# rubengooj/pl-slam

Measured on AMD Instinct MI355X. Metric: stereo pairs/sec (1500 ORB + 200 LBD BF-match), higher is better.
Workload: dtype fp4; 1 GPU; C2: synthetic 752x480 stereo stream, 1500 ORB + 200 LBD per image, ORB+LBD L<->R and prev<->curr, mutual + ratio (StVO::match), then StereoFrame's gates over the L<->R tables (config_kitti.yaml:25-...; mutual=True, distinct_batches_in_rotation=3, stereo_gates=True, kernel=k_scan_sym_mfma_i, mfma_form=0

## Files before the change

plslam_amd/build.py:

```python
from __future__ import annotations

import hashlib
import os
import shutil
import subprocess
from concurrent.futures import ThreadPoolExecutor

_HERE = os.path.dirname(os.path.abspath(__file__))
_ROOT = os.path.dirname(_HERE)
CSRC = os.path.join(_HERE, "csrc")
OUT = os.path.join(_HERE, "lib", "libplslam_hip.so")
LEGACY_OUT = os.path.join(_HERE, "lib", "libplslam_hip_legacy.so")
OBJ_DIR = os.path.join(_ROOT, "build", "obj")
SOURCES = ["hamming.hip", "hamming_mfma_g.hip", "hamming_mfma_h.hip", "hamming_mfma_i.hip", "lba.hip", "lba_assemble_rows.hip", "lba_plan.hip", "lba_schur.hip",
           "map2kf.hip", "lbd.hip", "median_desc.hip", "match_grid.hip", "match_grid_listers.hip", "match_grid_dense.hip", "match_grid_api.hip", "stereo_gates.hip", "pose_gn.hip", "lbd_float.hip", "bow.hip",
           "loop_closure.hip", "gba.hip", "pgo.hip", "local_map.hip", "map_insert.hip", "lc_fuse.hip",
           "context.hip", "match_plan.hip", "host_calls.hip", "match_pipeline.hip", "gather.hip"]
LEGACY_SOURCES = ["hamming_mfma.hip", "hamming_mfma_d.hip"]
LEGACY_AWARE = ("context.hip", "hamming_mfma_h.hip")
HEADERS = [os.path.join(CSRC, h) for h in ("common.hpp", "match_tables.hpp", "match_planner.hpp", "match_plan.hpp", "gfx950_only.hpp", "mfma_h_common.hpp", "lba_rows_dev.hpp", "lba_lists.hpp", "lba_blocks_dev.hpp", "lba_plan.hpp", "match_grid.hpp", "match_grid_layout.hpp", "match_grid_dev.hpp",
                                            "stereo_gates_dev.hpp", "pose_gn_dev.hpp", "se3_dev.hpp", "ldlt_dense_dev.hpp", "lookback_dev.hpp", "lc_fuse_plan.hpp")] + [os.path.join(_ROOT, "include", "plslam_hip.h")]
FLAGS = ["--offload-arch=gfx950", "-O3", "-std=c++17", "-fPIC", "-ffp-contract=off",
         "-Wall", "-Wextra", "-Wno-unused-command-line-argument",
         "-include", os.path.join(CSRC, "gfx950_only.hpp")]
PER_SOURCE_FLAGS = {"hamming_mfma_h.hip": ["-Wno-inline-asm"], "hamming_mfma_i.hip": ["-Wno-inline-asm"]}


def legacy_scans() -> bool:
    return os.environ.get("PLSLAM_BUILD_LEGACY_SCANS", "0") not in ("", "0")
# ... 94 lines not shown
```

plslam_amd/csrc/common.hpp:

```cpp
#pragma once

#include <hip/hip_runtime.h>
#include <stdint.h>

#include <cstdio>
#include <mutex>
#include <vector>

#include "match_tables.hpp"
#include "plslam_hip.h"

namespace plslam {

void set_last_error(const char* fmt, ...);

#define PLSLAM_HIP_CHECK(expr)                                                              \
    do {                                                                                    \
        hipError_t e_ = (expr);                                                             \
        if (e_ != hipSuccess) {                                                             \
            ::plslam::set_last_error("%s:%d: %s -> %s", __FILE__, __LINE__, #expr,           \
                                     hipGetErrorString(e_));                                \
            return e_ == hipErrorOutOfMemory ? PLSLAM_ENOMEM : PLSLAM_EHIP;                 \
        }                                                                                   \
    } while (0)
// ... 95 lines not shown
    hipDeviceProp_t prop;
    int scan_variant = PLSLAM_SCAN_AUTO;
    int scan_block = 0;
    int group_cap = 0;
    int sym_rows = 0;
    int mfma_form = 0;
    int col_split = 0;
    int exact_second = 0;
    int graph = 1;
    int post_workgroups = 0;
    int split_target = 0, split_min_tiles = 0;
    int split_post = 0;
    int post_xcd = 2;
    int zero_copy_kb = 64;
    int post_fuse = 0;
    int fuse = 0;
    std::mutex mu;
    plslam::DevBuf in_a, in_b, out_a, out_b, misc_a, misc_b, misc_c;
    plslam::HostBuf pin_in, pin_out;
    plslam::HostBuf pin_misc;
    plslam::LineRing lbd_ring;
    struct plslam_match_plan* host_plan = nullptr;
    struct plslam_match_plan* lc_plan = nullptr;
    plslam::DevBuf lc_in, lc_out, lc_tab;
    hipEvent_t lc_ev[2] = {nullptr, nullptr};
    plslam::DevBuf lc_args;
    std::vector<char> lc_args_h;
    int pgo_solver = 0;
    plslam::DevBuf pgo_scratch;
};
// ... 51 lines not shown
int sym_rows_per_partial(int rows_per_lane);
int launch_scan_sym(int rows_per_lane, const SymDesc* d_sym, const BlockDesc* d_blocks, int nblocks,
                    int32_t* d_zero, int nzero, hipStream_t s);
int launch_scan_sym_mfma(const SymDesc* d_sym, const BlockDesc* d_blocks, int nblocks, int32_t* d_zero,
                         int nzero, bool multi_window, bool directed, hipStream_t s);
int launch_scan_sym_mfma_g(const SymDesc* d_sym, const BlockDesc* d_blocks, int nblocks, int32_t* d_zero,
                           int nzero, bool multi_window, bool directed, bool fused, hipStream_t s);
int merge_partials16_cols(int parts);
int launch_merge_partials16(const SymDesc* d_sym, const BlockDesc* d_blocks, int nblocks, int parts, hipStream_t s);
int launch_split_post(const SymDesc* d_sym, const BlockDesc* d_blocks, int nblocks, int parts, const ProblemDesc* d_probs, hipStream_t s);
int launch_split_rows_dump(const ProblemDesc* d_probs, const BlockDesc* d_fin_blocks, int nblocks, hipStream_t s);
int launch_scan_sym_mfma_h(const SymDesc* d_sym, const BlockDesc* d_blocks, int nblocks, int32_t* d_zero, int nzero,
                           bool directed, hipStream_t s);
int launch_scan_sym_mfma_i(const SymDesc* d_sym, const BlockDesc* d_blocks, int nblocks, int32_t* d_zero, int nzero,
                           bool directed, hipStream_t s);
int merge_fix16_cols(int parts);
int launch_merge_fix16(const SymDesc* d_sym, const BlockDesc* d_blocks, int nblocks, int parts, bool fix, hipStream_t s, int grid_cap = 0);
int mh_slot_of_column(int n2, int j);
int launch_scan_dir_mfma(const SymDesc* d_sym, const BlockDesc* d_blocks, int nblocks, int32_t* d_zero, int nzero, hipStream_t s);
int launch_scan_mfma_form(int form, const SymDesc* d_sym, const BlockDesc* d_blocks, int nblocks, int32_t* d_zero,
                          int nzero, bool multi_window, bool directed, hipStream_t s, bool fused = false);
int launch_merge_partials(const SymDesc* d_sym, const BlockDesc* d_blocks, int nblocks, hipStream_t s);

int scan_rows_per_block(int variant, int block_threads);

int launch_gather_rows(const void* src, const int32_t* idx, int32_t n, int32_t row_bytes, void* dst,
                       hipStream_t s);

int launch_point_rows(const plslam_cam& K, double th, const double* T, const double* Xw,
                      const double* uv, const int32_t* lm, const int32_t* kf, int32_t nobs,
// ... 25 lines not shown
```

plslam_amd/csrc/context.hip:

```cpp
#include <stdarg.h>
#include <string.h>

#include <new>

#include "common.hpp"
#include "match_grid.hpp"
#include "match_plan.hpp"

namespace plslam {

static thread_local char g_err[512] = "";

void set_last_error(const char* fmt, ...)
{
    va_list ap;
    va_start(ap, fmt);
    vsnprintf(g_err, sizeof(g_err), fmt, ap);
    va_end(ap);
}

int DevBuf::reserve(size_t bytes)
{
    if (bytes <= cap) return PLSLAM_OK;
    if (p) {
// ... 133 lines not shown
}

namespace {
int g_legacy_scans = PLSLAM_BUILD_LEGACY_SCANS;
struct OptionDesc { const char* name; int plslam_ctx::*member; int* global; int lo, hi; };
const OptionDesc kOptions[] = {
    {"scan_variant", &plslam_ctx::scan_variant, nullptr, PLSLAM_SCAN_AUTO, PLSLAM_SCAN_MFMA},
    {"scan_block", &plslam_ctx::scan_block, nullptr, 0, 1024},
    {"sym_rows", &plslam_ctx::sym_rows, nullptr, 0, 4},
    {"group_cap", &plslam_ctx::group_cap, nullptr, 0, 64},
    {"mfma_form", &plslam_ctx::mfma_form, nullptr, 0, 5},
    {"legacy_scans", nullptr, &g_legacy_scans, 0, -1},
    {"fuse", &plslam_ctx::fuse, nullptr, 0, 2},
    {"post_fuse", &plslam_ctx::post_fuse, nullptr, 0, 2},
    {"exact_second", &plslam_ctx::exact_second, nullptr, 0, 1},
    {"col_split", &plslam_ctx::col_split, nullptr, 0, 2},
    {"graph", &plslam_ctx::graph, nullptr, 0, 2},
    {"grid_dense", nullptr, &plslam::g_grid_dense, 0, 1},
    {"zero_copy_kb", &plslam_ctx::zero_copy_kb, nullptr, -(1 << 20), 1 << 20},
    {"post_xcd", &plslam_ctx::post_xcd, nullptr, 0, 2},
    {"split_post", &plslam_ctx::split_post, nullptr, 0, 1},
    {"split_target", &plslam_ctx::split_target, nullptr, 0, 64},
    {"split_min_tiles", &plslam_ctx::split_min_tiles, nullptr, 0, 64},
    {"post_workgroups", &plslam_ctx::post_workgroups, nullptr, 0, INT32_MAX},
    {"pgo_solver", &plslam_ctx::pgo_solver, nullptr, 0, 1},
};
const OptionDesc* find_option(const char* key, bool to_write)
{
    for (const OptionDesc& o : kOptions)
        if (!strcmp(key, o.name) && (!to_write || o.lo <= o.hi)) return &o;
// ... 46 lines not shown
```

plslam_amd/csrc/match_plan.hip:

```cpp
#include <string.h>

#include <new>

#include "match_plan.hpp"

using namespace plslam;

static PlanOptions plan_options_of(const plslam_ctx* ctx)
{
    PlanOptions o;
    o.cu_count = ctx->prop.multiProcessorCount;
    o.scan_variant = ctx->scan_variant; o.scan_block = ctx->scan_block; o.sym_rows = ctx->sym_rows; o.group_cap = ctx->group_cap;
    o.mfma_form = ctx->mfma_form; o.col_split = ctx->col_split; o.exact_second = ctx->exact_second;
    o.split_target = ctx->split_target; o.split_min_tiles = ctx->split_min_tiles; o.split_post = ctx->split_post;
    o.post_xcd = ctx->post_xcd; o.post_fuse = ctx->post_fuse; o.fuse = ctx->fuse;
    o.rows_wpq = scan_rows_per_block(PLSLAM_SCAN_WAVE_PER_QUERY, 256);
    o.rows_lpq = scan_rows_per_block(PLSLAM_SCAN_LANE_PER_QUERY, ctx->scan_block ? ctx->scan_block : 256);
    const int lanes[3] = {1, 4, 16};
    for (int k = 0; k < 3; ++k) { o.merge16_cols[k] = merge_partials16_cols(lanes[k]); o.fix16_cols[k] = merge_fix16_cols(lanes[k]); }
    for (int k = 0; k < 2; ++k) { o.sym_block_rows[k] = sym_rows_per_block(lanes[k]); o.sym_partial_rows[k] = sym_rows_per_partial(lanes[k]); }
    return o;
}

bool plslam::ctx_takes_device_row_count(const plslam_ctx* ctx) { return plan_options_of(ctx).takes_device_row_count(); }

int plslam::plan_build(plslam_ctx* ctx, const plslam_match_problem* probs, int32_t nprob,
                       plslam_match_plan* P, const int32_t* n1_dev0)
{
    PlanChoice& c = P->choice;
    PlanTables& t = P->tab;
// ... 30 lines not shown
    if (!base) {
        if ((r = P->tables.reserve(t.total))) return r;
        base = P->tables.as<char>();
    }
    auto at = [&](int k) { return base + t.piece[k].off; };
    P->d_scans = reinterpret_cast<ScanDesc*>(at(PlanTables::SCANS));
    P->d_syms = reinterpret_cast<SymDesc*>(at(PlanTables::SYMS));
    P->d_probs = reinterpret_cast<ProblemDesc*>(at(PlanTables::PROBS));
    P->d_scan_blocks = reinterpret_cast<BlockDesc*>(at(PlanTables::SCAN_BLOCKS));
    P->d_sym_blocks = reinterpret_cast<BlockDesc*>(at(PlanTables::SYM_BLOCKS));
    P->d_merge_blocks = reinterpret_cast<BlockDesc*>(at(PlanTables::MERGE_BLOCKS));
    P->d_fin_blocks = reinterpret_cast<BlockDesc*>(at(PlanTables::FIN_BLOCKS));
    P->d_count_dst = reinterpret_cast<int32_t**>(at(PlanTables::COUNT_DST));
    P->d_dirs = reinterpret_cast<SymDesc*>(at(PlanTables::DIRS));
    P->d_dir_blocks = reinterpret_cast<BlockDesc*>(at(PlanTables::DIR_BLOCKS));
    P->ngate_blocks = 0;
    P->ngates = 0;

    if (!P->probs_in_place) PLSLAM_HIP_CHECK(hipMemcpyAsync(base, stg, t.total, hipMemcpyHostToDevice, ctx->stream));
    return PLSLAM_OK;
}

int plslam::plan_run(plslam_match_plan* P, hipStream_t s, hipStream_t sp)
{
    const bool split = sp != s;
    if (split) {
        if (!P->scan_done) PLSLAM_HIP_CHECK(hipEventCreateWithFlags(&P->scan_done, hipEventDisableTiming));
        if (!P->post_done) PLSLAM_HIP_CHECK(hipEventCreateWithFlags(&P->post_done, hipEventDisableTiming));
    }
    if (P->post_pending) {
// ... 3 lines not shown
    plslam_match_plan::Ev* ev = nullptr;
    if (P->profiling) {
        if (P->ev_used == P->evs.size()) {
            plslam_match_plan::Ev e{};
            PLSLAM_HIP_CHECK(hipEventCreate(&e.e0));
            PLSLAM_HIP_CHECK(hipEventCreate(&e.e1));
            PLSLAM_HIP_CHECK(hipEventCreate(&e.e2));
            P->evs.push_back(e);
        }
        ev = &P->evs[P->ev_used++];
        PLSLAM_HIP_CHECK(hipEventRecord(ev->e0, s));
    }
    const PlanChoice& c = P->choice;
    const PlanTables& t = P->tab;
    const int nsym_blocks = (int)t.sym_blocks.size(), ndir_blocks = (int)t.dir_blocks.size(), nscan_blocks = (int)t.scan_blocks.size();
    const int nmerge_blocks = (int)t.merge_blocks.size();
    int r;
    bool zeroed = false;
    if (c.fused) {
        PLSLAM_HIP_CHECK(hipMemsetAsync(P->d_counts_zero, 0, sizeof(int32_t) * (size_t)P->nprob, s));
        zeroed = true;
    }
    if (nsym_blocks > 0) {
        r = c.sym_mfma ? launch_scan_mfma_form(c.mfma_form, P->d_syms, P->d_sym_blocks, nsym_blocks, P->d_counts_zero,
                                               zeroed ? 0 : P->nprob, t.sym_mfma_multi, false, s, c.fused)
                       : launch_scan_sym(c.sym_rows, P->d_syms, P->d_sym_blocks, nsym_blocks, P->d_counts_zero, P->nprob, s);
        if (r) return r;
        zeroed = true;
    }
    if (ndir_blocks > 0) {
        r = launch_scan_mfma_form(c.mfma_form, P->d_dirs, P->d_dir_blocks, ndir_blocks, P->d_counts_zero,
                                  zeroed ? 0 : P->nprob, t.dir_multi, true, s, c.fused);
        if (r) return r;
        zeroed = true;
    }
    if (nscan_blocks > 0 || !zeroed) {
        r = launch_scan(P->ctx, c.scan_variant, c.block_threads, P->d_scans, P->d_scan_blocks, nscan_blocks, P->d_counts_zero,
                        zeroed ? 0 : P->nprob, s);
        if (r) return r;
    }
    if (ev) PLSLAM_HIP_CHECK(hipEventRecord(ev->e1, s));
// ... 309 lines not shown
```

plslam_amd/csrc/match_plan.hpp:

```cpp
#pragma once

#include "common.hpp"
#include "match_planner.hpp"

struct plslam_match_plan {
    plslam_ctx* ctx = nullptr;
    int32_t nprob = 0;
    plslam::PlanChoice choice;
    plslam::PlanTables tab;
    bool split_post = false;
    plslam::DevBuf keys, counts, partials;
    plslam::DevBuf rowtmp;
    plslam::DevBuf tables;
    std::vector<char> staging;
    plslam::HostBuf staging_pin;
    bool pin_tables = false;
    plslam::ScanDesc* d_scans = nullptr; plslam::SymDesc *d_syms = nullptr, *d_dirs = nullptr; plslam::ProblemDesc* d_probs = nullptr;
    plslam::BlockDesc *d_scan_blocks = nullptr, *d_sym_blocks = nullptr, *d_dir_blocks = nullptr, *d_merge_blocks = nullptr, *d_fin_blocks = nullptr;
    int32_t** d_count_dst = nullptr;
    int32_t* d_counts_zero = nullptr;
    plslam::DevBuf gate_tables;
    std::vector<char> gate_staging;
    bool probs_in_place = false;
    plslam_stereo_gate_problem* d_gates = nullptr;
    plslam::BlockDesc* d_gate_blocks = nullptr;
    int32_t ngate_blocks = 0, ngates = 0;
    int32_t* d_gate_counts = nullptr;
    bool profiling = false;
    hipGraphExec_t graph_exec = nullptr;
    bool graph_failed = false;
    void drop_graph() { if (graph_exec) (void)hipGraphExecDestroy(graph_exec); graph_exec = nullptr; graph_failed = false; }
    struct Ev { hipEvent_t e0, e1, e2; };
    std::vector<Ev> evs;
// ... 36 lines not shown
```

plslam_amd/csrc/match_planner.hpp:

```cpp
#pragma once

#include <algorithm>
#include <vector>

#include "match_tables.hpp"

namespace plslam {

struct PlanOptions {
    int cu_count = 0;
    int scan_variant = PLSLAM_SCAN_AUTO, scan_block = 0, sym_rows = 0, group_cap = 0, mfma_form = 0, col_split = 0, exact_second = 0;
    int split_target = 0, split_min_tiles = 0, split_post = 0, post_xcd = 2, post_fuse = 0, fuse = 0;
    int rows_wpq = 0, rows_lpq = 0;
    int sym_block_rows[2] = {0, 0};
    int sym_partial_rows[2] = {0, 0};
    int merge16_cols[3] = {0, 0, 0};
    int fix16_cols[3] = {0, 0, 0};

    bool takes_device_row_count() const
    {
        return (scan_variant == PLSLAM_SCAN_AUTO || scan_variant == PLSLAM_SCAN_MFMA) && (mfma_form == 0 || mfma_form == 2) &&
               col_split != 1 && split_post != 1 && fuse != 2;
    }
};

enum class ProblemPath : int32_t {
    empty,
    scan,
    sym,
    directed,
    split,
};

struct ProblemPlan {
    ProblemPath path;
    int32_t nsplit, cstep;
    int64_t key_row, part_row, tmp_row;
};

struct PlanChoice {
    PlanOptions opts;
    const char* error = nullptr;
    bool small = false;
    int scan_variant = 0, block_threads = 0;
    int rows_scan = 0;
    bool sym_mfma = false;
    bool dpair = false;
    int mfma_form = 0;
    int sym_rows = 1;
    int rows_sym = 0, rows_partial = 0;
    bool fused = false;
    bool col_split = false;
    bool split_post = false;
    bool exact_second = false;
    int merge_parts = 1;
    int merge_cols = 0;
    size_t group_cap = 2;
    int64_t key_rows = 0, part_rows = 0, tmp_rows = 0;
    bool counts_in_place = false, scatter_counts = false;
    std::vector<ProblemPlan> per;

    bool h_tables() const { return sym_mfma && mfma_form_is_h(mfma_form) && !fused; }
    bool partials16() const { return sym_mfma && mfma_form != 1; }
    bool lazy_keys() const { return h_tables() && !exact_second; }
    int64_t part_units(int32_t n1, int32_t n2) const
    {
        if (h_tables()) return (int64_t)((n1 + 255) / 256) * ((n2 + 255) / 256) * (exact_second ? 256 : 128);
        return (int64_t)((n1 + 63) / 64) * ((n2 + 255) / 256) * 128;
    }
};

#define PLSLAM_PLAN_REQUIRE(cond, code)   \
    do {                                  \
        if (!(cond)) {                    \
            c.error = #cond;              \
            return (code);                \
        }                                 \
    } while (0)

// ... 71 lines not shown
    const int32_t min_tiles = o.split_min_tiles > 0 ? o.split_min_tiles : 4;
    c.split_post = c.col_split && !c.h_tables() && !c.fused && o.split_post != 1 && nprob > 0;
    c.key_rows = c.part_rows = c.tmp_rows = 0;
    c.counts_in_place = nprob > 0;
    bool any_counter = false;
    for (int32_t i = 0; i < nprob; ++i) {
        const plslam_match_problem& p = probs[i];
        PLSLAM_PLAN_REQUIRE(p.n1 >= 0 && p.n2 >= 0, PLSLAM_EINVAL);
        PLSLAM_PLAN_REQUIRE(p.n1 == 0 || p.d1 != nullptr, PLSLAM_EINVAL);
        PLSLAM_PLAN_REQUIRE(p.n2 == 0 || p.d2 != nullptr, PLSLAM_EINVAL);
        PLSLAM_PLAN_REQUIRE(p.n1 == 0 || p.matches_12 != nullptr, PLSLAM_EINVAL);
        PLSLAM_PLAN_REQUIRE((reinterpret_cast<uintptr_t>(p.d1) & 3) == 0, PLSLAM_EINVAL);
        PLSLAM_PLAN_REQUIRE((reinterpret_cast<uintptr_t>(p.d2) & 3) == 0, PLSLAM_EINVAL);
        PLSLAM_PLAN_REQUIRE(p.n2 <= PLSLAM_MAX_TRAIN_ROWS, PLSLAM_ERANGE);
        PLSLAM_PLAN_REQUIRE(!p.mutual || p.n1 <= PLSLAM_MAX_TRAIN_ROWS, PLSLAM_ERANGE);
        ProblemPlan q{ProblemPath::empty, 1, 0, c.key_rows, c.part_rows, c.tmp_rows};
        const bool both = p.n1 > 0 && p.n2 > 0;
        if (c.col_split && both) {
            const int32_t tiles = (p.n2 + 31) / 32;
            const int32_t per = std::max((int32_t)((tiles + want - 1) / want), min_tiles);
            const int32_t ns = (tiles + per - 1) / per;
            if (ns > 1) { q.nsplit = ns; q.cstep = per * 32; }
        }
        q.path = q.nsplit > 1 ? ProblemPath::split : is_sym(p) ? ProblemPath::sym : c.sym_mfma && both ? ProblemPath::directed
                 : p.n1 > 0 ? ProblemPath::scan : ProblemPath::empty;
        c.key_rows += p.n1 + (p.mutual ? p.n2 : 0);
        if (q.path == ProblemPath::split) {
            for (int32_t s = 0; p.mutual && s < q.nsplit; ++s) c.part_rows += c.part_units(p.n1, std::min(q.cstep, p.n2 - s * q.cstep));
            c.tmp_rows += (int64_t)q.nsplit * p.n1;
        } else if (q.path == ProblemPath::sym) {
            c.part_rows += c.partials16() ? c.part_units(p.n1, p.n2) : (int64_t)((p.n1 + c.rows_partial - 1) / c.rows_partial) * p.n2;
        }
        c.split_post = c.split_post && is_sym(p) && !p.keep_prior;
        any_counter = any_counter || p.n_matches != nullptr;
        c.counts_in_place = c.counts_in_place && p.n_matches != nullptr && p.n_matches == probs[0].n_matches + i;
        c.per.push_back(q);
    }
    c.scatter_counts = any_counter && !c.counts_in_place;
    PLSLAM_PLAN_REQUIRE(c.key_rows < (int64_t(1) << 31), PLSLAM_ERANGE);
    if (has_n1_dev0 && !c.split_post) return PLSLAM_ENOTSUP;
    return PLSLAM_OK;
}
#undef PLSLAM_PLAN_REQUIRE

struct PlanBases {
    uint32_t* keys = nullptr;
    uint32_t* partials = nullptr;
    uint32_t* rowtmp = nullptr;
    int32_t* counts = nullptr;
    const int32_t* n1_dev0 = nullptr;
};

struct PlanTables {
    std::vector<ScanDesc> scans;
    std::vector<int32_t> scan_problem;
    std::vector<SymDesc> syms, dirs;
    std::vector<ProblemDesc> probs;
    std::vector<BlockDesc> scan_blocks, sym_blocks, dir_blocks, merge_blocks, fin_blocks;
    std::vector<int32_t*> user_counts;
    bool sym_mfma_multi = false, dir_multi = false;
    bool post_fused = false;
    size_t post_lds = 0;
    int32_t fin_row = 0;
    plslam_plan_info info{};
    enum { SCANS, SYMS, PROBS, SCAN_BLOCKS, SYM_BLOCKS, MERGE_BLOCKS, FIN_BLOCKS, COUNT_DST, DIRS, DIR_BLOCKS, NPIECES };
    struct Piece { const void* src; size_t bytes, off; } piece[NPIECES] = {};
    size_t total = 0;
    struct Group { int64_t cost; int32_t first, count; size_t xcd, at; };
    std::vector<Group> groups;
    std::vector<BlockDesc> dealt;
};

template <class KeyOf, class CostOf>
inline size_t deal_to_xcds(PlanTables& t, std::vector<BlockDesc>& blocks, size_t cap, KeyOf key_of, CostOf cost_of)
{
    t.groups.clear();
    for (size_t i = 0; i < blocks.size();) {
        size_t j = i;
        while (j < blocks.size() && j - i < cap && key_of(blocks[j]) == key_of(blocks[i])) ++j;
        t.groups.push_back({cost_of(blocks[i]), (int32_t)i, (int32_t)(j - i), 0, 0});
// ... 13 lines not shown
        x = (best + 1) & 7;
    }
    const size_t L = *std::max_element(len, len + 8);
    t.dealt.assign(8 * L, BlockDesc{-1, 0});
    for (const PlanTables::Group& g : t.groups)
        for (int32_t k = 0; k < g.count; ++k) t.dealt[g.xcd * L + g.at + (size_t)k] = blocks[(size_t)g.first + k];
    blocks.swap(t.dealt);
    return L;
}

inline void plan_tables(const PlanChoice& c, const plslam_match_problem* probs, const PlanBases& b, PlanTables& t)
{
    const int32_t nprob = (int32_t)c.per.size();
    t.scans.clear(); t.scan_problem.clear(); t.syms.clear(); t.dirs.clear(); t.probs.clear(); t.user_counts.clear();
    t.scan_blocks.clear(); t.sym_blocks.clear(); t.dir_blocks.clear(); t.merge_blocks.clear(); t.fin_blocks.clear();
    t.sym_mfma_multi = t.dir_multi = false;
    int64_t evals = 0, devals = 0, abytes = 0;
    auto blocks_of = [](std::vector<BlockDesc>& tab, size_t item, int32_t n, int32_t step) {
        for (int32_t r0 = 0; r0 < n; r0 += step) tab.push_back({(int32_t)item, r0});
    };
    for (int32_t i = 0; i < nprob; ++i) {
        const plslam_match_problem& p = probs[i];
        const ProblemPlan& q = c.per[(size_t)i];
        ProblemDesc pd{};
        pd.n1 = p.n1; pd.n2 = p.n2; pd.nnr = p.nnr; pd.mutual = p.mutual ? 1 : 0;
        pd.keep_prior = p.keep_prior ? 1 : 0;
        pd.matches_12 = p.matches_12;
        pd.n_matches = b.counts + i;
        t.user_counts.push_back(p.n_matches);
        uint32_t* k12 = b.keys + 2 * q.key_row;
// ... 31 lines not shown
                if (n2s > 2048) (p.mutual ? t.sym_mfma_multi : t.dir_multi) = true;
                dst.push_back(y);
            }
            evals += nn;
            devals += (p.mutual ? 2 : 1) * nn;
            abytes += p.mutual ? 2 * 32LL * (p.n1 + p.n2) + 16LL * (p.n1 + p.n2) : 32LL * (p.n1 + p.n2) + 16LL * p.n1;
            break;
        }
        case ProblemPath::sym:
            pd.lazy21 = c.lazy_keys();
            y.a = p.d1; y.b = p.d2; y.keys12 = k12; y.keys21 = k21;
            y.part21 = b.partials + 2 * q.part_row;
            pd.part21 = y.part21;
            y.n1 = p.n1; y.n2 = p.n2; y.n_iblk = (p.n1 + c.rows_partial - 1) / c.rows_partial;
            if (c.split_post) { y.mutual = i + 1; y.matches_12 = p.matches_12; y.n1_dev = b.n1_dev0; }
            if (c.fused) {
                y.mutual = 1; y.matches_12 = p.matches_12; y.n_matches = pd.n_matches; y.nnr = p.nnr;
                t.sym_blocks.push_back({(int32_t)t.syms.size(), 0});
            } else {
                blocks_of(t.sym_blocks, t.syms.size(), p.n1, c.rows_sym);
                if (c.partials16()) blocks_of(t.merge_blocks, t.syms.size(), (p.n2 + 31) & ~31, c.merge_cols);
                else blocks_of(t.merge_blocks, t.syms.size(), p.n2, 256);
            }
            if (c.sym_mfma && p.n2 > 2048) t.sym_mfma_multi = true;
            t.syms.push_back(y);
            evals += nn;
            devals += 2 * nn;
            abytes += 2 * 32LL * (p.n1 + p.n2) + 16LL * (p.n1 + p.n2);
            break;
        case ProblemPath::directed:
            for (int dir = 0; dir < (p.mutual ? 2 : 1); ++dir) {
// ... 21 lines not shown
                evals += nn;
                devals += nn;
                abytes += 32LL * (p.n1 + p.n2) + 16LL * sc.nq;
            }
            break;
        case ProblemPath::empty:
            break;
        }
        t.probs.push_back(pd);
    }
    auto item_of = [](const BlockDesc& e) { return e.item; };
    auto stream_cost = [&c](const std::vector<SymDesc>& d) {
        return [&c, &d](const BlockDesc& e) { return (int64_t)d[(size_t)e.item].n2 * (c.fused ? d[(size_t)e.item].n1 : 1); };
    };
    if (!t.sym_blocks.empty()) deal_to_xcds(t, t.sym_blocks, c.group_cap, item_of, stream_cost(t.syms));
    if (!t.dir_blocks.empty()) deal_to_xcds(t, t.dir_blocks, c.group_cap, item_of, stream_cost(t.dirs));
    if (c.scan_variant != PLSLAM_SCAN_WAVE_PER_QUERY && !t.scan_blocks.empty())
        deal_to_xcds(t, t.scan_blocks, c.group_cap, [&t](const BlockDesc& e) { return t.scan_problem[(size_t)e.item]; },
                     [&t](const BlockDesc& e) { return (int64_t)t.scans[(size_t)e.item].nt; });
    t.fin_row = 0;
    if (c.opts.post_xcd == 2 && t.fin_blocks.size() >= 64)
        t.fin_row = (int32_t)deal_to_xcds(t, t.fin_blocks, (size_t)-1, item_of, [](const BlockDesc&) { return (int64_t)0; });

    bool pf = c.opts.post_fuse == 2 && c.lazy_keys() && !c.col_split && nprob > 0;
    int32_t max_n2 = 0;
    for (int32_t i = 0; pf && i < nprob; ++i) {
        pf = c.per[(size_t)i].path == ProblemPath::sym && t.probs[(size_t)i].part21 != nullptr && probs[i].n2 <= POST_FUSED_MAX_N2 &&
             (probs[i].n1 + 255) / 256 <= POST_FUSED_MAX_ROW_BLOCKS;
        max_n2 = std::max(max_n2, probs[i].n2);
    }
    t.post_fused = pf;
    t.post_lds = pf ? sizeof(uint32_t) * 2 * (size_t)((max_n2 + 63) & ~63) : 0;

    const int32_t nsym = (int32_t)t.syms.size(), ndir = (int32_t)t.dirs.size();
    t.info.distance_evals = evals;
    t.info.directed_evals = devals;
    t.info.algorithmic_bytes = abytes;
    t.info.n_scans = (int32_t)t.scans.size() + 2 * nsym + ndir;
    t.info.scan_blocks = (int32_t)(t.scan_blocks.size() + t.sym_blocks.size() + t.dir_blocks.size());
    t.info.scan_variant = nsym ? (c.sym_mfma ? PLSLAM_SCAN_MFMA : PLSLAM_SCAN_SYMMETRIC) : (ndir ? PLSLAM_SCAN_MFMA : c.scan_variant);
    t.info.scan_block_threads = nsym ? (c.sym_rows == 4 && !c.sym_mfma ? 64 : 256) : (ndir ? 256 : c.block_threads);

    auto put = [&t](int k, const auto& v, size_t n) { t.piece[k] = {v.data(), n * sizeof(v[0]), 0}; };
    put(PlanTables::SCANS, t.scans, t.scans.size());
    put(PlanTables::SYMS, t.syms, t.syms.size());
    put(PlanTables::PROBS, t.probs, t.probs.size());
    put(PlanTables::SCAN_BLOCKS, t.scan_blocks, t.scan_blocks.size());
    put(PlanTables::SYM_BLOCKS, t.sym_blocks, t.sym_blocks.size());
    put(PlanTables::MERGE_BLOCKS, t.merge_blocks, t.merge_blocks.size());
    put(PlanTables::FIN_BLOCKS, t.fin_blocks, t.fin_blocks.size());
    put(PlanTables::COUNT_DST, t.user_counts, c.scatter_counts ? t.user_counts.size() : 0);
    put(PlanTables::DIRS, t.dirs, t.dirs.size());
    put(PlanTables::DIR_BLOCKS, t.dir_blocks, t.dir_blocks.size());
    t.total = 0;
    for (PlanTables::Piece& x : t.piece) { x.off = t.total; t.total += align256(x.bytes); }
    if (t.total == 0) t.total = 256;
}

}
```

Measured before the change: 1.743 million stereo pairs/s.

## Add single-workgroup symmetric MFMA scan kernel for small matching problems

Adds a dedicated kernel for symmetric (mutual) Hamming matching problems of at most 256x256 descriptors, such as the 200-line LBD sets. One 256-thread workgroup computes the whole distance tile with fp4 MFMA and produces row-wise keys (with an exact re-scan of the winning column group) and column-wise keys directly. This removes the partial-table writes and the separate merge/finalise stage for these problems. The planner routes qualifying problems to the new kernel, which is on by default (small_sym=0 maps to enabled), at the cost of another launch and a lot of hand-scheduled asm that is harder to check for correctness.

```diff
diff --git a/plslam_amd/build.py b/plslam_amd/build.py
--- a/plslam_amd/build.py
+++ b/plslam_amd/build.py
@@ -12,7 +12,7 @@
 OUT = os.path.join(_HERE, "lib", "libplslam_hip.so")
 LEGACY_OUT = os.path.join(_HERE, "lib", "libplslam_hip_legacy.so")
 OBJ_DIR = os.path.join(_ROOT, "build", "obj")
-SOURCES = ["hamming.hip", "hamming_mfma_g.hip", "hamming_mfma_h.hip", "hamming_mfma_i.hip", "lba.hip", "lba_assemble_rows.hip", "lba_plan.hip", "lba_schur.hip",
+SOURCES = ["hamming.hip", "hamming_mfma_g.hip", "hamming_mfma_h.hip", "hamming_mfma_i.hip", "hamming_mfma_s.hip", "lba.hip", "lba_assemble_rows.hip", "lba_plan.hip", "lba_schur.hip",
            "map2kf.hip", "lbd.hip", "median_desc.hip", "match_grid.hip", "match_grid_listers.hip", "match_grid_dense.hip", "match_grid_api.hip", "stereo_gates.hip", "pose_gn.hip", "lbd_float.hip", "bow.hip",
            "loop_closure.hip", "gba.hip", "pgo.hip", "local_map.hip", "map_insert.hip", "lc_fuse.hip",
            "context.hip", "match_plan.hip", "host_calls.hip", "match_pipeline.hip", "gather.hip"]
diff --git a/plslam_amd/csrc/common.hpp b/plslam_amd/csrc/common.hpp
--- a/plslam_amd/csrc/common.hpp
+++ b/plslam_amd/csrc/common.hpp
@@ -133,6 +133,7 @@
     int post_xcd = 2;
     int zero_copy_kb = 64;
     int post_fuse = 0;
+    int small_sym = 0;
     int fuse = 0;
     std::mutex mu;
     plslam::DevBuf in_a, in_b, out_a, out_b, misc_a, misc_b, misc_c;
@@ -214,6 +215,7 @@
                            bool directed, hipStream_t s);
 int launch_scan_sym_mfma_i(const SymDesc* d_sym, const BlockDesc* d_blocks, int nblocks, int32_t* d_zero, int nzero,
                            bool directed, hipStream_t s);
+int launch_scan_sym_small(const SymDesc* d_sym, const BlockDesc* d_blocks, int nblocks, int32_t* d_zero, int nzero, hipStream_t s);
 int merge_fix16_cols(int parts);
 int launch_merge_fix16(const SymDesc* d_sym, const BlockDesc* d_blocks, int nblocks, int parts, bool fix, hipStream_t s, int grid_cap = 0);
 int mh_slot_of_column(int n2, int j);
diff --git a/plslam_amd/csrc/context.hip b/plslam_amd/csrc/context.hip
--- a/plslam_amd/csrc/context.hip
+++ b/plslam_amd/csrc/context.hip
@@ -171,6 +171,7 @@
     {"fuse", &plslam_ctx::fuse, nullptr, 0, 2},
     {"post_fuse", &plslam_ctx::post_fuse, nullptr, 0, 2},
     {"exact_second", &plslam_ctx::exact_second, nullptr, 0, 1},
+    {"small_sym", &plslam_ctx::small_sym, nullptr, 0, 1},
     {"col_split", &plslam_ctx::col_split, nullptr, 0, 2},
     {"graph", &plslam_ctx::graph, nullptr, 0, 2},
     {"grid_dense", nullptr, &plslam::g_grid_dense, 0, 1},
diff --git a/plslam_amd/csrc/hamming_mfma_s.hip b/plslam_amd/csrc/hamming_mfma_s.hip
--- /dev/null
+++ b/plslam_amd/csrc/hamming_mfma_s.hip
@@ -0,0 +1,284 @@
+#include "mfma_h_common.hpp"
+
+namespace plslam {
+
+namespace {
+constexpr uint32_t MS_MAG = FP4_FOUR;
+constexpr uint32_t MS_ACC_BITS = 0x4B000000u + 4096u;
+constexpr uint32_t MS_KEY16_MAX = 0x3FFFu;
+constexpr uint32_t MS_COL_PENALTY = 0x4000u;
+constexpr uint32_t MS_NONE16 = 0x7BFFu;
+constexpr uint32_t MS_NONE32 = MS_NONE16 * 0x00010001u;
+constexpr int MS_MAX_TILES = 8;
+}
+
+#ifdef PLSLAM_MS_PROF
+constexpr int MS_PROF_WGS = 65536;
+__device__ unsigned long long g_ms_prof[MS_PROF_WGS * 4];
+#define PLSLAM_MS_TICK() __builtin_readcyclecounter()
+#endif
+
+__global__ void __launch_bounds__(256, 3)
+k_scan_sym_small(const SymDesc* __restrict__ syms, const BlockDesc* __restrict__ blocks, int32_t* __restrict__ zero, int nzero)
+{
+    constexpr int ROWX_STRIDE = 33;
+    constexpr int TILE_BYTES = MH_TILE_BYTES;
+    __shared__ __attribute__((aligned(16))) uint8_t bexp[MS_MAX_TILES * TILE_BYTES];
+    static_assert(sizeof(bexp) >= 4 * 64 * ROWX_STRIDE * 4, "the transpose must fit");
+    __shared__ __attribute__((aligned(16))) uint32_t braw[256 * 8];
+    __shared__ __attribute__((aligned(16))) uint32_t colstage[MS_MAX_TILES * 256];
+    static_assert(sizeof(bexp) + sizeof(braw) + sizeof(colstage) <= 53248, "three workgroups per CU");
+
+#ifdef PLSLAM_MS_PROF
+    const unsigned long long prof_t0 = PLSLAM_MS_TICK();
+#endif
+    if (blockIdx.x == 0)
+        for (int i = threadIdx.x; i < nzero; i += 256) zero[i] = 0;
+    asm volatile("s_setreg_imm32_b32 hwreg(HW_REG_MODE, 6, 2), 3");
+
+    const int wg = xcd_remap_(blockIdx.x, gridDim.x);
+    const BlockDesc bd = blocks[wg];
+    if (bd.item < 0) return;
+    const SymDesc sd = syms[bd.item];
+    const int n1 = sd.n1, n2 = sd.n2;
+    const int S = (n2 + 31) >> 5;
+    const int tid = threadIdx.x, lane = tid & 63;
+    const int w = __builtin_amdgcn_readfirstlane(tid >> 6);
+    const int c = lane & 31, g = lane >> 5;
+    const gcu32_t araw = (gcu32_t) reinterpret_cast<const uint32_t*>(sd.a);
+    const gcu32_t bglob = (gcu32_t) reinterpret_cast<const uint32_t*>(sd.b);
+
+    const int ej = tid >> 3, ewd = tid & 7;
+    uint32_t raw[MS_MAX_TILES];
+#pragma unroll
+    for (int t = 0; t < MS_MAX_TILES; ++t) {
+        raw[t] = 0;
+        if (t < S) {
+            const int j = S * ej + t, jc = j < n2 ? j : n2 - 1;
+            raw[t] = bglob[jc * 8 + ewd];
+        }
+    }
+    uint32_t aw[2][MH_KSTEPS];
+#pragma unroll
+    for (int mt = 0; mt < 2; ++mt) {
+        const int row = 128 * mt + 32 * w + 16 * ((c >> 2) & 1) + (c & 3) + 4 * (c >> 3);
+        const int rrow = row < n1 ? row : n1 - 1;
+        const gcu32_t p = araw + (size_t)rrow * 8 + g;
+#pragma unroll
+        for (int ks = 0; ks < MH_KSTEPS; ++ks) aw[mt][ks] = p[2 * ks];
+    }
+#pragma unroll
+    for (int t = 0; t < MS_MAX_TILES; ++t) {
+        if (t < S) {
+            const int j = S * ej + t;
+            i32x4 v = expand_dword_fp4<false, MS_MAG>(raw[t]);
+            if (j < n2) braw[j * 8 + ewd] = raw[t];
+            else v = i32x4{0, 0, 0, 0};
+            *reinterpret_cast<i32x4*>(bexp + t * TILE_BYTES + ej * MH_ROW_STRIDE + ewd * 16) = v;
+        }
+    }
+    i32x4 afrag[2][MH_KSTEPS];
+#pragma unroll
+    for (int mt = 0; mt < 2; ++mt)
+#pragma unroll
+        for (int ks = 0; ks < MH_KSTEPS; ++ks) afrag[mt][ks] = expand_dword_fp4<true, MS_MAG>(aw[mt][ks]);
+
+    uint32_t gm[16];
+#pragma unroll
+    for (int s = 0; s < 16; ++s) gm[s] = MS_NONE32;
+    u32x16 seed;
+#pragma unroll
+    for (int r = 0; r < 16; ++r) seed[r] = MS_ACC_BITS + (uint32_t)(16 * g + r);
+    asm volatile("" : "+v"(seed));
+    int lim = n2 - S * c;
+    lim = lim < 0 ? 0 : (lim > S ? S : lim);
+    const int lim_part = n2 % S;
+
+    __syncthreads();
+#ifdef PLSLAM_MS_PROF
+    const unsigned long long prof_t1 = PLSLAM_MS_TICK();
+#endif
+
+#define PLSLAM_MS_EPI2(ACC, MT, Q)                                                                 \
+    {                                                                                              \
+        asm("v_pk_minimum3_f16 %0, %0, %1, %2 op_sel:[0,0,1] op_sel_hi:[1,1,0]" : "+v"(gm[8 * (MT) + (Q)]) : "v"(ACC[Q]), "v"(ACC[(Q) + 8])); \
+        asm("v_pk_minimum3_f16 %0, %0, %1, %2 op_sel:[0,0,1] op_sel_hi:[1,1,0]" : "+v"(gm[8 * (MT) + (Q) + 1]) : "v"(ACC[(Q) + 1]), "v"(ACC[(Q) + 9])); \
+        if ((Q) == 0) asm("v_min_f32 %0, %1, %2" : "=v"(cfa) : "v"(ACC[Q]), "v"(ACC[(Q) + 8]));    \
+        else asm("v_min3_f32 %0, %0, %1, %2" : "+v"(cfa) : "v"(ACC[Q]), "v"(ACC[(Q) + 8]));        \
+        asm("v_min3_f32 %0, %0, %1, %2" : "+v"(cfa) : "v"(ACC[(Q) + 1]), "v"(ACC[(Q) + 9]));       \
+        __builtin_amdgcn_sched_barrier(0);                                                         \
+    }
+#define PLSLAM_MS_MMA(ACC, MT, KS, CIN)                                                            \
+    {                                                                                              \
+        const i32x8 a8 = {afrag[MT][KS].x, afrag[MT][KS].y, afrag[MT][KS].z, afrag[MT][KS].w, 0, 0, 0, 0}; \
+        const i32x8 b8 = {bfr[KS].x, bfr[KS].y, bfr[KS].z, bfr[KS].w, 0, 0, 0, 0};                 \
+        ACC = __builtin_amdgcn_mfma_scale_f32_32x32x64_f8f6f4(a8, b8, CIN, 4, 4, 0, 0, 0, 0);      \
+        asm volatile("" : "+v"(ACC));                      \
+        __builtin_amdgcn_sched_barrier(0);                                                         \
+    }
+    f32x16 m1;
+    {
+        u32x16 none;
+#pragma unroll
+        for (int r = 0; r < 16; ++r) asm volatile("v_mov_b32 %0, %1" : "=v"(none[r]) : "s"(MS_NONE32));
+        m1 = __builtin_bit_cast(f32x16, none);
+    }
+    uint32_t cm0_prev = MS_NONE32;
+    uint32_t* const cstage = colstage + 64 * w + lane;
+    const uint8_t* bt = bexp + c * MH_ROW_STRIDE + 16 * g;
+
+    __builtin_amdgcn_s_setprio(1);
+#pragma unroll 1
+    for (int t = 0; t < S; ++t, bt += TILE_BYTES) {
+        i32x4 bfr[MH_KSTEPS];
+#pragma unroll
+        for (int ks = 0; ks < MH_KSTEPS; ++ks) bfr[ks] = *reinterpret_cast<const i32x4*>(bt + 32 * ks);
+        if (t == 0 || t == lim_part) {
+            const uint32_t pen = lim == t ? MS_COL_PENALTY : 0u;
+#pragma unroll
+            for (int r = 0; r < 16; ++r) seed[r] += pen;
+            asm volatile("" : "+v"(seed));
+        }
+        const f32x16 cseed = __builtin_bit_cast(f32x16, seed);
+        f32x16 m0;
+        float cfa = 0.0f;
+        __builtin_amdgcn_sched_barrier(0);
+        PLSLAM_MS_MMA(m0, 0, 0, cseed)
+        asm volatile("s_nop 1");
+        __builtin_amdgcn_sched_barrier(0);
+        PLSLAM_MS_EPI2(m1, 1, 0) PLSLAM_MS_MMA(m0, 0, 1, m0)
+        PLSLAM_MS_EPI2(m1, 1, 2) PLSLAM_MS_MMA(m0, 0, 2, m0)
+        PLSLAM_MS_EPI2(m1, 1, 4) PLSLAM_MS_MMA(m0, 0, 3, m0)
+        PLSLAM_MS_EPI2(m1, 1, 6)
+        const uint32_t cm1 = __builtin_bit_cast(uint32_t, cfa);
+        if (t > 0) cstage[(t - 1) * 256] = __builtin_amdgcn_perm(cm1, cm0_prev, 0x05040100u);
+        __builtin_amdgcn_sched_barrier(0);
+        asm volatile("v_mfma_f32_32x32x64_f8f6f4 %0, %1, %2, %3 cbsz:4 blgp:4" : "=&v"(m1) : "v"(afrag[1][0]), "v"(bfr[0]), "v"(cseed));
+        asm volatile("s_nop 7");
+        __builtin_amdgcn_sched_barrier(0);
+        PLSLAM_MS_EPI2(m0, 0, 0)
+        PLSLAM_MS_MMA(m1, 1, 1, m1)    PLSLAM_MS_EPI2(m0, 0, 2)
+        PLSLAM_MS_MMA(m1, 1, 2, m1)    PLSLAM_MS_EPI2(m0, 0, 4)
+        PLSLAM_MS_MMA(m1, 1, 3, m1)    PLSLAM_MS_EPI2(m0, 0, 6)
+        cm0_prev = __builtin_bit_cast(uint32_t, cfa);
+    }
+    {
+        float cfa = 0.0f;
+        asm volatile("s_nop 7\n\ts_nop 7");
+        __builtin_amdgcn_sched_barrier(0);
+        PLSLAM_MS_EPI2(m1, 1, 0) PLSLAM_MS_EPI2(m1, 1, 2) PLSLAM_MS_EPI2(m1, 1, 4) PLSLAM_MS_EPI2(m1, 1, 6)
+        cstage[(S - 1) * 256] = __builtin_amdgcn_perm(__builtin_bit_cast(uint32_t, cfa), cm0_prev, 0x05040100u);
+    }
+    __builtin_amdgcn_s_setprio(0);
+#undef PLSLAM_MS_EPI2
+#undef PLSLAM_MS_MMA
+#ifdef PLSLAM_MS_PROF
+    const unsigned long long prof_t2 = PLSLAM_MS_TICK();
+#endif
+    __syncthreads();
+
+    const int row = 32 * w + lane + (lane & 32) * 3;
+    u32x4_t a_lo = {0, 0, 0, 0}, a_hi = {0, 0, 0, 0};
+    if (row < n1) {
+        const gcu32x4_t ap = (gcu32x4_t)(araw + (size_t)row * 8);
+        a_lo = ap[0];
+        a_hi = ap[1];
+    }
+
+    {
+        const int ct = tid >> 5, cc = tid & 31, j = S * cc + ct;
+        if (ct < S && j < n2) {
+            uint32_t b0 = 0xFFFFFFFFu, b1 = 0xFFFFFFFFu;
+#pragma unroll
+            for (int q = 0; q < 8; ++q) {
+                const uint32_t word = colstage[ct * 256 + 32 * q + cc];
+                const int base = 16 * q;
+                if (base < n1) {
+                    const uint32_t k16 = word & 0xFFFFu, k = ((k16 >> 5) << 8) | (uint32_t)(base + (int)(k16 & 15u));
+                    b1 = umin_(b1, umax_(b0, k));
+                    b0 = umin_(b0, k);
+                }
+                if (base + 128 < n1) {
+                    const uint32_t k16 = word >> 16, k = ((k16 >> 5) << 8) | (uint32_t)(base + 128 + (int)(k16 & 15u));
+                    b1 = umin_(b1, umax_(b0, k));
+                    b0 = umin_(b0, k);
+                }
+            }
+            const uint32_t k0 = ((b0 >> 8) << KEY_IDX_BITS) | (b0 & 255u);
+            const uint32_t k1 = (b1 >> 8) <= 256u ? (((b1 >> 8) << KEY_IDX_BITS) | KEY_IDX_MASK) : KEY_NONE;
+            ((gu2_t) reinterpret_cast<u32x2_t*>(sd.keys21))[j] = u32x2_t{k0, k1};
+        }
+    }
+
+    uint32_t* rowx = reinterpret_cast<uint32_t*>(bexp) + w * (64 * ROWX_STRIDE);
+#pragma unroll
+    for (int s = 0; s < 16; ++s) {
+        const int lrow = 32 * (s >> 3) + 16 * g + (s & 7);
+        rowx[lrow * ROWX_STRIDE + c] = gm[s] & 0xFFE0u;
+        rowx[(lrow + 8) * ROWX_STRIDE + c] = (gm[s] >> 16) & 0xFFE0u;
+    }
+    __builtin_amdgcn_fence(__ATOMIC_RELEASE, "wavefront");
+    __builtin_amdgcn_wave_barrier();
+    __builtin_amdgcn_fence(__ATOMIC_ACQUIRE, "wavefront");
+    if (row < n1) {
+        uint32_t k0 = 0xFFFFFFFFu, k1 = 0xFFFFFFFFu;
+        const uint32_t* mine = rowx + lane * ROWX_STRIDE;
+#pragma unroll
+        for (int cls = 0; cls < 32; ++cls) {
+            uint32_t x;
+            asm("v_lshl_or_b32 %0, %1, 16, %2" : "=v"(x) : "v"(mine[cls]), "n"(cls));
+            asm("v_med3_u32 %0, %1, %2, %0" : "+v"(k1) : "v"(k0), "v"(x));
+            k0 = umin_(k0, x);
+        }
+        uint32_t r0 = KEY_NONE, r1 = KEY_NONE;
+        if ((k0 >> 16) <= MS_KEY16_MAX) {
+            const uint32_t jb = (uint32_t)S * (k0 & 31u);
+            const uint32_t nvalid = umin_((uint32_t)S, (uint32_t)n2 - jb);
+            const uint32_t* rb = braw + jb * 8;
+            uint32_t bk = 0xFFFFFFFFu, sk = 0xFFFFFFFFu;
+#pragma unroll
+            for (int k = 0; k < MS_MAX_TILES; ++k) {
+                if (k < S) {
+                    const uint32_t kk = (uint32_t)k < nvalid ? (uint32_t)k : nvalid - 1u;
+                    const gvec4_t bl = *reinterpret_cast<const gvec4_t*>(rb + 8 * kk), bh = *reinterpret_cast<const gvec4_t*>(rb + 8 * kk + 4);
+                    const u32x4_t b_lo = {bl.x, bl.y, bl.z, bl.w}, b_hi = {bh.x, bh.y, bh.z, bh.w};
+                    const uint32_t d = hamming256(a_lo, a_hi, b_lo, b_hi);
+                    const uint32_t x = (uint32_t)k < nvalid ? ((d << 4) | (uint32_t)k) : 0xFFFFFFFFu;
+                    asm("v_med3_u32 %0, %1, %2, %0" : "+v"(sk) : "v"(bk), "v"(x));
+                    bk = umin_(bk, x);
+                }
+            }
+            r0 = ((bk >> 4) << KEY_IDX_BITS) | (jb + (bk & 15u));
+            const uint32_t in2 = sk == 0xFFFFFFFFu ? KEY_NONE : (((sk >> 4) << KEY_IDX_BITS) | (jb + (sk & 15u)));
+            r1 = (k1 >> 16) <= MS_KEY16_MAX ? umin_(in2, ((k1 >> 21) << KEY_IDX_BITS) | ((uint32_t)S * (k1 & 31u))) : in2;
+        }
+        ((gu2_t) reinterpret_cast<u32x2_t*>(sd.keys12))[row] = u32x2_t{r0, r1};
+    }
+#ifdef PLSLAM_MS_PROF
+    if (threadIdx.x == 0 && blockIdx.x < MS_PROF_WGS) {
+        const unsigned long long t3 = PLSLAM_MS_TICK();
+        g_ms_prof[4 * blockIdx.x + 0] = prof_t1 - prof_t0;
+        g_ms_prof[4 * blockIdx.x + 1] = prof_t2 - prof_t1;
+        g_ms_prof[4 * blockIdx.x + 2] = t3 - prof_t2;
+        g_ms_prof[4 * blockIdx.x + 3] = ((unsigned long long)S << 40) | (t3 - prof_t0);
+    }
+#endif
+}
+
+#ifdef PLSLAM_MS_PROF
+extern "C" int plslam_debug_k1s_profile(unsigned long long* out, int nwg)
+{
+    if (nwg > MS_PROF_WGS) nwg = MS_PROF_WGS;
+    return hipMemcpyFromSymbol(out, HIP_SYMBOL(g_ms_prof), sizeof(unsigned long long) * 4 * (size_t)nwg) == hipSuccess ? nwg : -1;
+}
+#endif
+
+int launch_scan_sym_small(const SymDesc* d_sym, const BlockDesc* d_blocks, int nblocks, int32_t* d_zero, int nzero, hipStream_t s)
+{
+    if (nblocks <= 0) return PLSLAM_OK;
+    hipLaunchKernelGGL(k_scan_sym_small, dim3(nblocks), dim3(256), 0, s, d_sym, d_blocks, d_zero, nzero);
+    PLSLAM_HIP_CHECK(hipGetLastError());
+    return PLSLAM_OK;
+}
+
+}
diff --git a/plslam_amd/csrc/match_plan.hip b/plslam_amd/csrc/match_plan.hip
--- a/plslam_amd/csrc/match_plan.hip
+++ b/plslam_amd/csrc/match_plan.hip
@@ -14,6 +14,7 @@
     o.mfma_form = ctx->mfma_form; o.col_split = ctx->col_split; o.exact_second = ctx->exact_second;
     o.split_target = ctx->split_target; o.split_min_tiles = ctx->split_min_tiles; o.split_post = ctx->split_post;
     o.post_xcd = ctx->post_xcd; o.post_fuse = ctx->post_fuse; o.fuse = ctx->fuse;
+    o.small_sym = ctx->small_sym != 1;
     o.rows_wpq = scan_rows_per_block(PLSLAM_SCAN_WAVE_PER_QUERY, 256);
     o.rows_lpq = scan_rows_per_block(PLSLAM_SCAN_LANE_PER_QUERY, ctx->scan_block ? ctx->scan_block : 256);
     const int lanes[3] = {1, 4, 16};
@@ -74,6 +75,7 @@
     P->d_count_dst = reinterpret_cast<int32_t**>(at(PlanTables::COUNT_DST));
     P->d_dirs = reinterpret_cast<SymDesc*>(at(PlanTables::DIRS));
     P->d_dir_blocks = reinterpret_cast<BlockDesc*>(at(PlanTables::DIR_BLOCKS));
+    P->d_small_blocks = reinterpret_cast<BlockDesc*>(at(PlanTables::SMALL_BLOCKS));
     P->ngate_blocks = 0;
     P->ngates = 0;
 
@@ -107,7 +109,7 @@
     const PlanChoice& c = P->choice;
     const PlanTables& t = P->tab;
     const int nsym_blocks = (int)t.sym_blocks.size(), ndir_blocks = (int)t.dir_blocks.size(), nscan_blocks = (int)t.scan_blocks.size();
-    const int nmerge_blocks = (int)t.merge_blocks.size();
+    const int nmerge_blocks = (int)t.merge_blocks.size(), nsmall_blocks = (int)t.small_blocks.size();
     int r;
     bool zeroed = false;
     if (c.fused) {
@@ -118,6 +120,11 @@
         r = c.sym_mfma ? launch_scan_mfma_form(c.mfma_form, P->d_syms, P->d_sym_blocks, nsym_blocks, P->d_counts_zero,
                                                zeroed ? 0 : P->nprob, t.sym_mfma_multi, false, s, c.fused)
                        : launch_scan_sym(c.sym_rows, P->d_syms, P->d_sym_blocks, nsym_blocks, P->d_counts_zero, P->nprob, s);
+        if (r) return r;
+        zeroed = true;
+    }
+    if (nsmall_blocks > 0) {
+        r = launch_scan_sym_small(P->d_syms, P->d_small_blocks, nsmall_blocks, P->d_counts_zero, zeroed ? 0 : P->nprob, s);
         if (r) return r;
         zeroed = true;
     }
diff --git a/plslam_amd/csrc/match_plan.hpp b/plslam_amd/csrc/match_plan.hpp
--- a/plslam_amd/csrc/match_plan.hpp
+++ b/plslam_amd/csrc/match_plan.hpp
@@ -17,6 +17,7 @@
     bool pin_tables = false;
     plslam::ScanDesc* d_scans = nullptr; plslam::SymDesc *d_syms = nullptr, *d_dirs = nullptr; plslam::ProblemDesc* d_probs = nullptr;
     plslam::BlockDesc *d_scan_blocks = nullptr, *d_sym_blocks = nullptr, *d_dir_blocks = nullptr, *d_merge_blocks = nullptr, *d_fin_blocks = nullptr;
+    plslam::BlockDesc* d_small_blocks = nullptr;
     int32_t** d_count_dst = nullptr;
     int32_t* d_counts_zero = nullptr;
     plslam::DevBuf gate_tables;
diff --git a/plslam_amd/csrc/match_planner.hpp b/plslam_amd/csrc/match_planner.hpp
--- a/plslam_amd/csrc/match_planner.hpp
+++ b/plslam_amd/csrc/match_planner.hpp
@@ -11,6 +11,7 @@
     int cu_count = 0;
     int scan_variant = PLSLAM_SCAN_AUTO, scan_block = 0, sym_rows = 0, group_cap = 0, mfma_form = 0, col_split = 0, exact_second = 0;
     int split_target = 0, split_min_tiles = 0, split_post = 0, post_xcd = 2, post_fuse = 0, fuse = 0;
+    bool small_sym = false;
     int rows_wpq = 0, rows_lpq = 0;
     int sym_block_rows[2] = {0, 0};
     int sym_partial_rows[2] = {0, 0};
@@ -35,6 +36,7 @@
 struct ProblemPlan {
     ProblemPath path;
     int32_t nsplit, cstep;
+    bool small_sym = false;
     int64_t key_row, part_row, tmp_row;
 };
 
@@ -63,6 +65,10 @@
     bool h_tables() const { return sym_mfma && mfma_form_is_h(mfma_form) && !fused; }
     bool partials16() const { return sym_mfma && mfma_form != 1; }
     bool lazy_keys() const { return h_tables() && !exact_second; }
+    bool takes_small_sym(int32_t n1, int32_t n2) const
+    {
+        return opts.small_sym && lazy_keys() && opts.post_fuse != 2 && n1 >= 1 && n1 <= 256 && n2 >= 1 && n2 <= 256;
+    }
     int64_t part_units(int32_t n1, int32_t n2) const
     {
         if (h_tables()) return (int64_t)((n1 + 255) / 256) * ((n2 + 255) / 256) * (exact_second ? 256 : 128);
@@ -164,7 +170,7 @@
         PLSLAM_PLAN_REQUIRE((reinterpret_cast<uintptr_t>(p.d2) & 3) == 0, PLSLAM_EINVAL);
         PLSLAM_PLAN_REQUIRE(p.n2 <= PLSLAM_MAX_TRAIN_ROWS, PLSLAM_ERANGE);
         PLSLAM_PLAN_REQUIRE(!p.mutual || p.n1 <= PLSLAM_MAX_TRAIN_ROWS, PLSLAM_ERANGE);
-        ProblemPlan q{ProblemPath::empty, 1, 0, c.key_rows, c.part_rows, c.tmp_rows};
+        ProblemPlan q{ProblemPath::empty, 1, 0, false, c.key_rows, c.part_rows, c.tmp_rows};
         const bool both = p.n1 > 0 && p.n2 > 0;
         if (c.col_split && both) {
             const int32_t tiles = (p.n2 + 31) / 32;
@@ -178,6 +184,8 @@
         if (q.path == ProblemPath::split) {
             for (int32_t s = 0; p.mutual && s < q.nsplit; ++s) c.part_rows += c.part_units(p.n1, std::min(q.cstep, p.n2 - s * q.cstep));
             c.tmp_rows += (int64_t)q.nsplit * p.n1;
+        } else if (q.path == ProblemPath::sym && c.takes_small_sym(p.n1, p.n2)) {
+            q.small_sym = true;
         } else if (q.path == ProblemPath::sym) {
             c.part_rows += c.partials16() ? c.part_units(p.n1, p.n2) : (int64_t)((p.n1 + c.rows_partial - 1) / c.rows_partial) * p.n2;
         }
@@ -207,13 +215,14 @@
     std::vector<SymDesc> syms, dirs;
     std::vector<ProblemDesc> probs;
     std::vector<BlockDesc> scan_blocks, sym_blocks, dir_blocks, merge_blocks, fin_blocks;
+    std::vector<BlockDesc> small_blocks;
     std::vector<int32_t*> user_counts;
     bool sym_mfma_multi = false, dir_multi = false;
     bool post_fused = false;
     size_t post_lds = 0;
     int32_t fin_row = 0;
     plslam_plan_info info{};
-    enum { SCANS, SYMS, PROBS, SCAN_BLOCKS, SYM_BLOCKS, MERGE_BLOCKS, FIN_BLOCKS, COUNT_DST, DIRS, DIR_BLOCKS, NPIECES };
+    enum { SCANS, SYMS, PROBS, SCAN_BLOCKS, SYM_BLOCKS, MERGE_BLOCKS, FIN_BLOCKS, COUNT_DST, DIRS, DIR_BLOCKS, SMALL_BLOCKS, NPIECES };
     struct Piece { const void* src; size_t bytes, off; } piece[NPIECES] = {};
     size_t total = 0;
     struct Group { int64_t cost; int32_t first, count; size_t xcd, at; };
@@ -257,6 +266,7 @@
     const int32_t nprob = (int32_t)c.per.size();
     t.scans.clear(); t.scan_problem.clear(); t.syms.clear(); t.dirs.clear(); t.probs.clear(); t.user_counts.clear();
     t.scan_blocks.clear(); t.sym_blocks.clear(); t.dir_blocks.clear(); t.merge_blocks.clear(); t.fin_blocks.clear();
+    t.small_blocks.clear();
     t.sym_mfma_multi = t.dir_multi = false;
     int64_t evals = 0, devals = 0, abytes = 0;
     auto blocks_of = [](std::vector<BlockDesc>& tab, size_t item, int32_t n, int32_t step) {
@@ -318,7 +328,10 @@
             pd.part21 = y.part21;
             y.n1 = p.n1; y.n2 = p.n2; y.n_iblk = (p.n1 + c.rows_partial - 1) / c.rows_partial;
             if (c.split_post) { y.mutual = i + 1; y.matches_12 = p.matches_12; y.n1_dev = b.n1_dev0; }
-            if (c.fused) {
+            if (q.small_sym) {
+                y.part21 = nullptr; pd.part21 = nullptr;
+                t.small_blocks.push_back({(int32_t)t.syms.size(), 0});
+            } else if (c.fused) {
                 y.mutual = 1; y.matches_12 = p.matches_12; y.n_matches = pd.n_matches; y.nnr = p.nnr;
                 t.sym_blocks.push_back({(int32_t)t.syms.size(), 0});
             } else {
@@ -370,6 +383,7 @@
         return [&c, &d](const BlockDesc& e) { return (int64_t)d[(size_t)e.item].n2 * (c.fused ? d[(size_t)e.item].n1 : 1); };
     };
     if (!t.sym_blocks.empty()) deal_to_xcds(t, t.sym_blocks, c.group_cap, item_of, stream_cost(t.syms));
+    if (!t.small_blocks.empty()) deal_to_xcds(t, t.small_blocks, c.group_cap, item_of, stream_cost(t.syms));
     if (!t.dir_blocks.empty()) deal_to_xcds(t, t.dir_blocks, c.group_cap, item_of, stream_cost(t.dirs));
     if (c.scan_variant != PLSLAM_SCAN_WAVE_PER_QUERY && !t.scan_blocks.empty())
         deal_to_xcds(t, t.scan_blocks, c.group_cap, [&t](const BlockDesc& e) { return t.scan_problem[(size_t)e.item]; },
@@ -393,7 +407,7 @@
     t.info.directed_evals = devals;
     t.info.algorithmic_bytes = abytes;
     t.info.n_scans = (int32_t)t.scans.size() + 2 * nsym + ndir;
-    t.info.scan_blocks = (int32_t)(t.scan_blocks.size() + t.sym_blocks.size() + t.dir_blocks.size());
+    t.info.scan_blocks = (int32_t)(t.scan_blocks.size() + t.sym_blocks.size() + t.dir_blocks.size() + t.small_blocks.size());
     t.info.scan_variant = nsym ? (c.sym_mfma ? PLSLAM_SCAN_MFMA : PLSLAM_SCAN_SYMMETRIC) : (ndir ? PLSLAM_SCAN_MFMA : c.scan_variant);
     t.info.scan_block_threads = nsym ? (c.sym_rows == 4 && !c.sym_mfma ? 64 : 256) : (ndir ? 256 : c.block_threads);
 
@@ -408,6 +422,7 @@
     put(PlanTables::COUNT_DST, t.user_counts, c.scatter_counts ? t.user_counts.size() : 0);
     put(PlanTables::DIRS, t.dirs, t.dirs.size());
     put(PlanTables::DIR_BLOCKS, t.dir_blocks, t.dir_blocks.size());
+    put(PlanTables::SMALL_BLOCKS, t.small_blocks, t.small_blocks.size());
     t.total = 0;
     for (PlanTables::Piece& x : t.piece) { x.off = t.total; t.total += align256(x.bytes); }
     if (t.total == 0) t.total = 256;
```

Result: faster. 1.768 million stereo pairs/s (median of 6 runs) (+1.5%).
